# jrl-umi3218/jrl-walkgen

Measured on AMD Instinct MI355X. Metric: QP-MPC ticks/sec (batch=4096, N=16), higher is better.
Workload: dtype f64

## Files before the change

### jrl-walkgen_amd/csrc/wg_capi.hip

```cpp
#include <hip/hip_runtime.h>

#include <climits>
#include <cmath>
#include <cstdarg>
#include <cstdio>
#include <cstdlib>
#include <cstring>
#include <limits>
#include <memory>
#include <mutex>
#include <string>
#include <type_traits>
#include <vector>

#include "../../include/wg_mpc.h"
#include "wg_ql_device.hpp"
#include "wg_tick_device.hpp"
#include "wg_tick_kernels.hpp"
#include "wg_pldp_device.hpp"
#include "wg_dimitrov_device.hpp"
#include "wg_preview_device.hpp"
#include "wg_gramian_device.hpp"
#include "wg_zmpdisc_device.hpp"
#include "wg_footcons_device.hpp"
// ... 586 lines not shown
  if (!model) return fail(WG_ERR_BAD_ARG, "null model");
  if (model->N < 2 || model->N > wg::kNMaxH) return fail(WG_ERR_BAD_ARG, "N=%d outside [2,%d]", model->N, wg::kNMaxH);
  if ((int)(model->T / model->Tctrl) != WG_SAMPLES_PER_TICK)
    return fail(WG_ERR_BAD_ARG, "T/Tctrl must be %d", WG_SAMPLES_PER_TICK);
  if (tick_max_prw_steps(*model) > wg::kSMax)
    return fail(WG_ERR_BAD_ARG, "step_period=%g: a horizon of N=%d instants of T=%g previews up to %d steps, the tick holds %d",
                model->step_period, model->N, model->T, tick_max_prw_steps(*model), wg::kSMax);
  const size_t lds = TickPlan(*model).lds;
  if (lds > 160 * 1024) return fail(WG_ERR_TOO_LARGE, "tick needs %zu B of LDS > 160 KiB", lds);
  std::vector<double> qb;
  if (model->flags & (WG_FLAG_GRAMIAN_MFMA_F64 | WG_FLAG_GRAMIAN_MFMA_F32)) {
    qb.resize((size_t)model->N * model->N);
    const int prec = (model->flags & WG_FLAG_GRAMIAN_MFMA_F32) ? WG_GRAMIAN_F32 : WG_GRAMIAN_F64;
    if (int rc = wg_gramian_batch_ctx(ctx, 1, model->N, &model->T, &model->com_height_qp, model->alpha, model->beta, model->gamma,
                                  prec, qb.data()))
      return rc;
  }
  std::lock_guard<std::mutex> lk(ctx->mu);
  std::unique_ptr<wg::TickTables> host_tables_p(new wg::TickTables);
  wg::TickTables &host_tables = *host_tables_p;
  wg::build_tables(*model, host_tables, qb.empty() ? nullptr : qb.data());
  if (!host_tables.blocks_ok && !qb.empty())
    return fail(WG_ERR_BAD_ARG, "the matrix-core Gramian is not positive definite enough for ql0002's factorisation");
  if (!ctx->tables_dev) HIP_TRY(hipMalloc(reinterpret_cast<void **>(&ctx->tables_dev), sizeof(wg::TickTables)));
  if (!ctx->model_dev) HIP_TRY(hipMalloc(reinterpret_cast<void **>(&ctx->model_dev), sizeof(wg_model_t)));
  if (int rc = ctx_wait_own(ctx)) return rc;
  HostScope hs(ctx);
  WG_H2D(ctx->tables_dev, &host_tables, sizeof host_tables);
  WG_H2D(ctx->model_dev, model, sizeof(wg_model_t));
  WG_HOST_WAIT();
  ctx->model = *model;
  ctx->model_set = true;
  return WG_OK;
}

size_t wg_mpc_tick_lds_bytes_for(const wg_model_t *model) {
  if (!model || model->N < 2 || model->N > wg::kNMaxH || tick_max_prw_steps(*model) > wg::kSMax) return 0;
  return TickPlan(*model).lds;
}

size_t wg_mpc_tick_lds_bytes_ctx(wg_ctx_t *ctx) {
  if (!ctx || !ctx->model_set) return 0;
  return TickPlan(ctx->model).lds;
}

int wg_mpc_reserve_ctx(wg_ctx_t *ctx, int max_gaits) {
// ... 1380 lines not shown
```

### jrl-walkgen_amd/csrc/wg_prof.hpp

```cpp
#pragma once
#include <hip/hip_runtime.h>

namespace wg {

enum ProfSlot : int {
  PS_NORMS = 0, PS_DIAGCHK = 1, PS_CHOL = 2 , PS_INVERSE = 3,
  PS_RESID = 4, PS_ZTWW_RESID = 5, PS_XSHIFT = 6, PS_BACKSUB_RESID = 7, PS_XMAG_RESID = 8,
  PS_SCAN = 9, PS_FDIFF = 10, PS_NEWNORMAL = 11, PS_SWEEP = 12, PS_ROUTE = 13, PS_STEP_PRE = 14, PS_BACKSUB_STEP = 15,
  PS_PICKDROP = 16, PS_STEP = 17, PS_ADD = 18, PS_XMAG_ADD = 19, PS_TAIL = 20,
  PS_RESET_BODY = 24, PS_RESID_GRAD = 25, PS_RESID_FWD = 26, PS_RESID_GX = 27,
  PS_N_ROUTE = 28, PS_N_COORD = 29, PS_N_DEPENDENT = 30, PS_BORDER_ROWS = 31,
  PS_SW_NORMS = 32, PS_SW_COEFF = 33, PS_SW_ROWS = 34,
  PS_TICK_PRE = 21, PS_TICK_ASSEMBLY = 22, PS_TICK_POST = 23,
  PS_TICK_LOAD = 35, PS_TICK_FSM = 36, PS_TICK_ORIENT = 37, PS_TICK_INSTANTS = 38,
  PS_TICK_COM = 39, PS_TICK_TRUNK = 40, PS_TICK_FEET = 41, PS_TICK_QUEUE = 42,
  PS_COUNT = 48
};

#ifdef WG_PROFILE
__device__ unsigned long long g_prof[PS_COUNT];

struct PtState {
  unsigned long long acc[28] = {0}, cnt[4] = {0}, sw[3] = {0};
  unsigned long long last = clock64();
};
#define PT_DECL PtState pt;
#define PT_PARAM , PtState &pt
#define PT_ARG , pt
#define PT(k) do { unsigned long long t_ = clock64(); pt.acc[k] += t_ - pt.last; pt.last = t_; } while (0)
#define PT_VIA(k, mem, reg) do { mem = reg; PT(k); reg = mem; } while (0)
#define PT_FLUSH do { if ((threadIdx.x & 63) == 0) { for (int k_ = 0; k_ < 28; ++k_) if (k_ < PS_TICK_PRE || k_ > PS_TICK_POST) atomicAdd(&g_prof[k_], pt.acc[k_]); \
                                                      for (int k_ = 0; k_ < 4; ++k_) atomicAdd(&g_prof[PS_N_ROUTE + k_], pt.cnt[k_]); \
                                                      for (int k_ = 0; k_ < 3; ++k_) atomicAdd(&g_prof[PS_SW_NORMS + k_], pt.sw[k_]); } } while (0)
#define PT_SW_PARAM , unsigned long long *ptsw = nullptr
#define PT_SW_ARG , pt.sw
#define PT_SW(k) do { if (ptsw) { unsigned long long t_ = clock64(); ptsw[(k) - PS_SW_NORMS] += t_ - ptsw_last; ptsw_last = t_; } } while (0)
#define PT_SW_BEGIN unsigned long long ptsw_last = clock64();
#define PT_COUNT(k) do { pt.cnt[(k) - PS_N_ROUTE]++; } while (0)
#define PT_LOCAL_BEGIN unsigned long long ptl_last = clock64();
#define PT_LOCAL(k) do { unsigned long long t_ = clock64(); if ((threadIdx.x & 63) == 0) atomicAdd(&g_prof[k], t_ - ptl_last); ptl_last = t_; } while (0)

struct TkState {
  unsigned long long acc[PS_COUNT] = {0};
  unsigned long long last = clock64();
};
#define TK_DECL TkState tk;
#define TK(k) do { unsigned long long t_ = clock64(); tk.acc[k] += t_ - tk.last; tk.last = t_; } while (0)
#define TK_RESTART do { tk.last = clock64(); } while (0)
#define TK_ADD_(k) atomicAdd(&g_prof[k], tk.acc[k])
#define TK_FLUSH do { if ((threadIdx.x & 63) == 0) { const unsigned long long store_ = clock64() - tk.last; \
    TK_ADD_(PS_TICK_LOAD); TK_ADD_(PS_TICK_FSM); TK_ADD_(PS_TICK_ORIENT); TK_ADD_(PS_TICK_INSTANTS); TK_ADD_(PS_TICK_ASSEMBLY); \
    TK_ADD_(PS_TICK_COM); TK_ADD_(PS_TICK_TRUNK); TK_ADD_(PS_TICK_FEET); TK_ADD_(PS_TICK_QUEUE); \
    atomicAdd(&g_prof[PS_TICK_PRE], tk.acc[PS_TICK_LOAD] + tk.acc[PS_TICK_FSM] + tk.acc[PS_TICK_ORIENT] + tk.acc[PS_TICK_INSTANTS]); \
    atomicAdd(&g_prof[PS_TICK_POST], tk.acc[PS_TICK_COM] + tk.acc[PS_TICK_TRUNK] + tk.acc[PS_TICK_FEET] + tk.acc[PS_TICK_QUEUE] + store_); } } while (0)
#else
#define PT_DECL
#define PT_PARAM
#define PT_ARG
#define PT(k) do {} while (0)
#define PT_VIA(k, mem, reg) ((void)0)
#define PT_FLUSH do {} while (0)
#define PT_SW_PARAM
#define PT_SW_ARG
#define PT_SW(k) do {} while (0)
#define PT_SW_BEGIN
#define PT_COUNT(k) do {} while (0)
#define PT_LOCAL_BEGIN
#define PT_LOCAL(k) ((void)0)
#define TK_DECL
#define TK(k) ((void)0)
#define TK_RESTART ((void)0)
#define TK_FLUSH ((void)0)
#endif

}
```

### jrl-walkgen_amd/csrc/wg_ql_device.hpp

```cpp
#pragma once
#include <hip/hip_runtime.h>

#include <type_traits>

#include "wg_wave.hpp"
#include "wg_ql_view.hpp"
#include "wg_ql_phases.hpp"

namespace wg {

#define WG_BACKSUB(q, s, nact, lane)                                                                   \
  do {                                                                                                 \
    if constexpr (P::kNM > 0 && P::kNM + 12 <= 48) backsub_lds<48>(q, s, nact, lane, q.sc0);          \
    else if (P::kNM == 0 && (P::kWideN || q.n >= 48) && (nact) <= 60) backsub_lds<96>(q, s, nact, lane, q.sc0);     \
    else if (P::kNM == 0 && !P::kRowOps && q.n >= 24 && (nact) <= 36) backsub_lds<48>(q, s, nact, lane, q.sc0); \
    else backsub(q, s, nact, lane);                                                                    \
  } while (0)
#define WG_SWEEP(q, s, nu, nact, lane) \
  do { if (P::kNM > 0 || (!P::kRowOps && q.n <= 64)) sweep_flat<P::kFixedLdz>(q, s, nu, nact, lane PT_SW_ARG); else sweep<(P::kRowOps ? WG_ELEM_GRP : 8), P::kWideN>(q, s, nu, nact, lane); } while (0)

#define QL_SCAN_ACCEPT                                                                        \
  if (wak <= 0.0) continue;                                                                   \
  double sumx = -sum * wak;                                                                   \
  if (k + 1 <= me) sumx = fabs(sumx);                                                         \
  if (sumx <= 0.0) continue;                                                                  \
  if (bidx >= 0 && sumx <= bestv) continue;                                                   \
  double tempa = temp + fabs(sum);                                                            \
  if (tempa <= temp) continue;                                                                \
  temp += onha * fabs(sum);                                                                   \
  if (temp <= tempa) continue;                                                                \
  bestv = sumx; bestres = sum; bestw = wak; bidx = k + 1
template <class P>
__device__ __forceinline__ QlResult ql_solve(const QlView &q, P &prob, double vsmall, int *hist, int hist_cap, QlResume *rs = nullptr) {
  constexpr bool kNan = P::kNanExact && (WG_NAN_REGIME != 0);
  int lane = wg_lane();
  const int n = q.n, m = q.m, me = q.me, mn = q.mn;
  QlResult out;
  out.hist_len = 0;
  const bool resuming = rs != nullptr && rs->valid != 0;
  int nact = 0, info = 0, iterc = 1, itref = 0, iflag = 0;
  const int maxit = (m + n) * 40;
  const double onha = 1.5, xmagr = .01, diagr = 2.0;
  const int ifinc = 3, kfinc = n > 10 ? n : 10;
  int jfinc = -kfinc;
  double xmag = 0.0, vfact = 1.0, res = 0.0, ratio = 0.0, diag = 0.0;
  double wsel = 1.0;
  int knext = 0;
  const int s_tail = q.r_tail;
  double *s = q.R + s_tail;
  bool early_exit = false;
  bool cap_hit = false;
  bool x_suspect = false;
  auto x_has_non_numbers = [&]() {
    bool b = false;
    for (int i = lane; i < n; i += 64) { const bool bi = !wg_sane(q.x[i]); b = b || bi; }
    return __ballot(b) != 0ull;
  };
  PT_DECL
  if (resuming) {
    nact = rs->nact; info = rs->info; iterc = rs->iterc; itref = rs->itref; iflag = rs->iflag; jfinc = rs->jfinc; knext = rs->knext;
    out.hist_len = rs->hist_len;
    xmag = rs->xmag; vfact = rs->vfact; res = rs->res; ratio = rs->ratio; diag = rs->diag;
    if constexpr (kNan) x_suspect = x_has_non_numbers();
  }

#define LOG_EVENT(code)                                                   \
  do {                                                                    \
    if (lane == 0 && hist && out.hist_len < hist_cap) hist[out.hist_len] = (code); \
    out.hist_len++;                                                       \
  } while (0)

  if (!resuming) {
    int fatal = 0x7fffffff;
    if constexpr (P::kCompact) {
      fatal = prob.norms(q, lane);
    } else {
      for (int k = lane; k < m; k += 64) {
        double sum = 0.0;
        if constexpr (P::kRowOps) sum = prob.row_sqnorm(q, k);
        else {
          WG_UNROLL
          for (int i = 0; i < n; ++i) { double a = Am(k, i); sum += a * a; }
        }
        if (sum > 0.0) sum = 1.0 / sqrt(sum);
        else if (q.b[k] == 0.0) {}
        else if (k + 1 <= me || !(q.b[k] <= 0.0)) fatal = k + 1 < fatal ? k + 1 : fatal;
        q.wa[k] = sum;
      }
    }
    for (int k = lane; k < n; k += 64) q.wa[m + k] = 1.0;
    fatal = uni(wave_min_int(fatal));
    if (fatal != 0x7fffffff) { info = -fatal; early_exit = true; }
  }
// ... 221 lines not shown
      if (nact != n) {
        if (P::kWideN || (P::kNM == 0 && n > 64 && n <= 128)) {
          double r0, r1;
          z_rows_times<(P::kRowOps ? WG_ELEM_GRP : 8)>(q, s, nact, n, lane, r0, r1);
          q.x[lane] -= r0;
          if (lane + 64 < n) q.x[lane + 64] -= r1;
        } else
        for (int i = lane; i < n; i += 64) {
          double sum = 0.0;
          WG_UNROLL
          for (int j = nact; j < n; ++j) sum += Zm(i, j) * s[j];
          q.x[i] -= sum;
        }
        info = 0;
        WG_WSYNC();
      }
      PT(PS_XSHIFT);
      if (nact != 0) {
        WG_BACKSUB(q, s, nact, lane);
        for (int k = lane; k < nact; k += 64) q.lam[k] += q.ww[k];
        WG_WSYNC();
      }
      PT(PS_BACKSUB_RESID);
      { double sm = 0.0; WG_REP(6) { sm = uni(xmag_sum(q, prob, vfact, lane)); WG_SINK(sm); } xmag = maxd(xmag, sm); }
      PT(PS_XMAG_RESID);
      if (iflag == itref) { st = ST_RESID; continue; }
      int kd = 0x7fffffff;
      for (int k = lane; k < nact; k += 64)
        if (!(q.lam[k] >= 0.0) && q.iact[k] > me) { kd = k < kd ? k : kd; }
      kd = uni(wave_min_int(kd));
      if (kd != 0x7fffffff) {
        LOG_EVENT(-q.iact[kd]);
        nact = drop_constraint(q, kd, nact, nact, lane);
        st = ST_RESID;
        continue;
      }
      if constexpr (kNan) x_suspect = x_suspect || x_has_non_numbers();
      st = ST_SCAN;
    }

    if (st == ST_SCAN) {
      next_scan: asm volatile("" : "+v"(lane));
      double bestv = 0.0, bestres = 0.0, bestw = 0.0;
      int bidx = -1;
      if (kNan && x_suspect) {
        if constexpr (kNan) {
// ... 271 lines not shown
        else zt_times_ww<P::kNM, (P::kRowOps ? WG_ELEM_GRP : 8), P::kWideN>(q, s, lane);
      } else {
        int k1 = knext - m;
        double sg = 1.0;
        if (k1 > n) { k1 = knext - mn; sg = -1.0; }
        for (int i = lane; i < n; i += 64) {
          q.ww[i] = (i == k1 - 1) ? sg : 0.0;
          double z = Zm(k1 - 1, i);
          s[i] = (sg > 0.0) ? z : -z;
        }
        WG_WSYNC();
      }
      PT(PS_NEWNORMAL);
      double parnew = 0.0, parinc = 0.0, step = 0.0, sumy;
      int kdrop = -1;
      int route;
      if (nact == n) route = 1;
      else {
        WG_SWEEP(q, s, n, nact, lane);
        PT(PS_SWEEP);
        if (nact == 0) route = 0;
        else {
          double suma = 0.0, sumb = 0.0, sumc = 0.0;
          WG_REP(5) {
          if constexpr (P::kNM > 0) {
            constexpr int NM = P::kNM;
            {
              const int il = lane < NM ? lane : NM - 1;
              const bool in = il < n;
              const int ic = in ? il : n - 1;
              const double zv = Zm(ic, nact), wv = q.ww[ic];
              const double zi = in ? zv : 0.0, wi = in ? wv : 0.0;
              q.sc0[il] = wi * zi; q.sc1[il] = fabs(wi * zi); q.sc2[il] = zi * zi;
            }
            WG_WSYNC();
            typedef __attribute__((address_space(3))) double lds_f64;
            const lds_f64 *src = (const lds_f64 *)(q.sc0 + (lane < 3 ? lane : 0) * (int)(q.sc1 - q.sc0));
            asm volatile("" : "+v"(src));
            double acc = 0.0;
#pragma unroll
            for (int i0 = 0; i0 < NM; i0 += kOsChunk) {
              double t[kOsChunk];
#pragma unroll
              for (int i = 0; i < kOsChunk; ++i) if (i0 + i < NM) t[i] = src[i0 + i];
#pragma unroll
              for (int i = 0; i < kOsChunk; ++i) if (i0 + i < NM) acc += t[i];
            }
            suma = rl(acc, 0); sumb = rl(acc, 1); sumc = rl(acc, 2);
            WG_WSYNC();
          } else {
            for (int i = lane; i < n; i += 64) {
              const double zi = Zm(i, nact), wi = q.ww[i];
              q.sc0[i] = wi * zi; q.sc1[i] = fabs(wi * zi); q.sc2[i] = zi * zi;
            }
            WG_WSYNC();
            const double *src = q.sc0 + (lane < 3 ? lane : 0) * (int)(q.sc1 - q.sc0);
            double acc = 0.0;
            int i = 0;
            for (; i + 8 <= n; i += 8) {
              double t[8];
#pragma unroll
              for (int e = 0; e < 8; ++e) t[e] = src[i + e];
#pragma unroll
              for (int e = 0; e < 8; ++e) acc += t[e];
            }
            for (; i < n; ++i) acc += src[i];
            suma = rl(acc, 0); sumb = rl(acc, 1); sumc = rl(acc, 2);
            WG_WSYNC();
          }
          WG_SINK(suma); WG_SINK(sumb); WG_SINK(sumc);
          }
          if (WG_UBOOL(!significant(sumb, fabs(suma)) || !(sumb > wg_kconst(vsmall)))) route = 1;
          else {
            sumc = sqrt(sumc);
            if (knext <= m) sumc /= wsel;
            if (WG_UBOOL(significant(sumc, fabs(suma)))) route = 0;
            else {
              PT_COUNT(PS_N_COORD);
              WG_BACKSUB(q, s, nact, lane);
              route = independent_coordinate(q, prob, knext, nact, vsmall, lane) ? 0 : 2;
            }
          }
        }
      }
      route = uni(route);
      PT(PS_ROUTE);
      PT_COUNT(PS_N_ROUTE);
      if (route != 0) PT_COUNT(PS_N_DEPENDENT);
      if (route != 0) {
        if (route == 1) WG_BACKSUB(q, s, nact, lane);
        kdrop = pick_drop<(P::kNM > 0), kNan>(q, nact, res, ratio, lane);
        info = -knext;
        if (kdrop < 0) { st = ST_CONVERGED; continue; }
        parinc = ratio;
        parnew = parinc;
// ... 49 lines not shown
          LOG_EVENT(-q.iact[kdrop]);
          nact = drop_constraint(q, kdrop, nu, nact, lane);
          double *snew = s - (nact + 1);
          if (nu > n) nu = n;
          for (int i0 = 0; i0 < nu; i0 += 64) {
            int i = i0 + lane;
            double v = (i < nu) ? s[i] : 0.0;
            WG_WSYNC();
            if (i < nu) snew[i] = v;
            WG_WSYNC();
          }
          s = snew;
          WG_SWEEP(q, s, nu, nact, lane);
        }
      }

      PT(PS_STEP);
      ql_activate(q, nact, knext, parnew, wsel, lane, n, mn);
      nact++;
      LOG_EVENT(knext);
      WG_WSYNC();
      PT(PS_ADD);
      double sm = 0.0;
      WG_REP(6) { sm = uni(xmag_sum(q, prob, vfact, lane)); WG_SINK(sm); }
      xmag = maxd(xmag, sm);
      PT(PS_XMAG_ADD);
      if (WG_UBOOL(sm < wg_kconst(xmagr) * xmag)) st = ST_RESET;
      else if (itref <= 0) st = ST_SCAN;
      else st = ST_RESID;
      if (q.nact_cap > 0 && nact > q.nact_cap) { cap_hit = true; break; }
      if (st == ST_SCAN) goto next_scan;
      continue;
    }

    if (st == ST_CONVERGED) {
      ++itref;
      jfinc = -1;
      if (itref == 1) { st = ST_RESID; continue; }
      st = ST_FINISH;
    }
  }
#undef LOG_EVENT

  PT(PS_TAIL);
  PT_FLUSH;
  if (cap_hit) {
    if (rs) {
      rs->nact = nact; rs->info = info; rs->iterc = iterc; rs->itref = itref; rs->iflag = iflag; rs->jfinc = jfinc; rs->knext = knext;
      rs->st = st; rs->hist_len = out.hist_len;
      rs->xmag = xmag; rs->vfact = vfact; rs->res = res; rs->ratio = ratio; rs->diag = diag;
    }
    out.ifail = kQlCapHit; out.n_iter = iterc; out.nact = nact;
    return out;
  }
  out.ifail = ql_ifail_of(info);
  out.n_iter = iterc;
  out.nact = nact;
  return out;
}

}
```

### jrl-walkgen_amd/csrc/wg_ql_herdt.hpp

```cpp
#pragma once
#include "wg_ql_device.hpp"

namespace wg {

constexpr int kSMaxQ = 4;
constexpr int kGvLd = 4;
constexpr int kQbLd = 32;

template <int NH, int NS>
__device__ __forceinline__ bool herdt_border_rows(const QlView &q, const double *gd, const double *Gv, double vsmall, int lane) {
  constexpr int M2 = 2 * NH;
  const int i = lane;
  const bool jerk = i < NH, foot = i >= NH && i < NH + NS, row = jerk || foot;
  const int fi = i - NH;
  const int gi = jerk ? i : M2 + (foot ? fi : 0);
  double acc[NS];
#pragma unroll
  for (int f = 0; f < NS; ++f)
    acc[f] = (jerk || (foot && f >= fi)) ? ((foot && f == fi) ? gd[gi] : Gv[gi * kGvLd + f]) : 0.0;
  const double dreg = jerk ? Rf(i, i) : 1.0;
  const int colbase = jerk ? i * (i + 1) / 2 : 0;
  const int khi = jerk ? i : 0;
  double rnext = (0 < khi) ? q.Rf[colbase] : 0.0;
  for (int k = 0; k < NH; ++k) {
// ... 152 lines not shown
#pragma unroll
  for (int t = 0; t < TZ; ++t) {
    const int e = lane + 64 * t;
    if (e < NH * NH) {
      const int i = e % NH, j = e / NH;
      Zm(i, j) = zv[t]; Zm(NH + i, NH + j) = zv[t];
      Zm(NH + i, j) = 0.0;
      Zm(i, NH + j) = ((z2sign[e >> 6] >> (e & 63)) & 1ull) ? wg_kconst(-0.0) : 0.0;
    }
  }
  for (int e = lane; e < (n - M2) * M2; e += 64) { const int i = M2 + e % (n - M2), j = e / (n - M2); Zm(i, j) = 0.0; }
}

template <int NH>
struct HerdtProb {
  static constexpr bool kCompact = true;
  static constexpr bool kNanExact = WG_TICK_NAN_EXACT != 0;
  static constexpr bool kHasFactor = true;
  static constexpr bool kRowOps = false;
  static constexpr int kNM = 2 * NH + 2 * 2;
  static constexpr int kCopRows = 4 * NH;
  static constexpr bool kWideN = false;
  static constexpr int kFixedLdz = kNM | 1;
  static_assert(4 * NH == 64, "one CoP row per lane needs 4N == 64");
  const double *Qb;
  const double *u;
  double *Gv;
  double *gd;
  const double *rowA, *rowB;
  const int *rowK, *stepidx;
  const double *V_f;
  const double *R2, *Z2;
  const unsigned long long *z2sign;
  double diag_b;
  int blocks_ok;
  int ns;
  double ax[NH], ay[NH];
  int fj;
  double ra, rb;
  double bcop;
  double ga, gb; int gk;
  __device__ __forceinline__ double fa() const { return ra + 0.0; }
  __device__ __forceinline__ double fb() const { return rb + 0.0; }
  struct FootRow { double v[4]; int c[4]; };
  __device__ __forceinline__ FootRow foot_row() const {
    const bool used = gk >= 0, pred = gk > 0;
    const int kk = used ? gk : 0;
    FootRow r;
    const int c1 = 2 * NH + kk, c3 = 2 * NH + ns + kk;
    r.c[0] = used ? (pred ? c1 - 1 : c1) : 2 * NH; r.c[1] = used ? c1 : 2 * NH;
    r.c[2] = used ? (pred ? c3 - 1 : c3) : 2 * NH; r.c[3] = used ? c3 : 2 * NH;
    r.v[0] = pred ? ga + 0.0 : 0.0; r.v[1] = used ? 0.0 - ga : 0.0;
    r.v[2] = pred ? gb + 0.0 : 0.0; r.v[3] = used ? 0.0 - gb : 0.0;
    return r;
  }

  __device__ __forceinline__ double G(const QlView &q, int i, int j) const {
    if (i == j) return gd[i];
    if (j < i) { const int t = i; i = j; j = t; }
// ... 511 lines not shown
```

### jrl-walkgen_amd/csrc/wg_ql_phases.hpp

```cpp
#pragma once
#include <hip/hip_runtime.h>

#include <type_traits>

#include "wg_wave.hpp"
#include "wg_ql_view.hpp"

namespace wg {

#ifndef WG_ELEM_GRP
#define WG_ELEM_GRP 4
#endif

__device__ __forceinline__ double sqrt_1to2(double x) {
  const double y = __builtin_amdgcn_rsq(x);
  double g = x * y;
  double h = y * 0.5;
  const double r = __builtin_fma(-h, g, 0.5);
  g = __builtin_fma(g, r, g);
  h = __builtin_fma(h, r, h);
  double d = __builtin_fma(-g, g, x);
  g = __builtin_fma(d, h, g);
  d = __builtin_fma(-g, g, x);
  g = __builtin_fma(d, h, g);
// ... 322 lines not shown


#ifndef WG_OS_CHUNK
#define WG_OS_CHUNK 12
#endif
constexpr int kOsChunk = WG_OS_CHUNK;
template <int NM>
__device__ __forceinline__ double ordered_sum_lds(double term, double *scratch, int cnt, int lane) {
  {
    const double v = (lane < cnt) ? term : 0.0;
    const double vl = rl(v, NM - 1);
    scratch[lane < NM ? lane : NM - 1] = lane < NM ? v : vl;
  }
  WG_WSYNC();
  double sum = 0.0;
#pragma unroll
  for (int i0 = 0; i0 < NM; i0 += kOsChunk) {
    double t[kOsChunk];
#pragma unroll
    for (int i = 0; i < kOsChunk; ++i) t[i] = (i0 + i < NM) ? scratch[i0 + i] : 0.0;
#pragma unroll
    for (int i = 0; i < kOsChunk; ++i) if (i0 + i < NM) sum += t[i];
  }
  WG_WSYNC();
  return sum;
}

template <int kLdzC = 0>
__device__ __forceinline__ void sweep_flat(const QlView &q, double *s, int nu, int nact, int lane PT_SW_PARAM) {
  const int n = q.n;
  if (nu - 1 <= nact) return;
  PT_SW_BEGIN
  double *chain = q.sc2;
  WG_REP(3)
  if (sweep_range_ok<true>(s, nact, nu, lane)) {
    double cur = s[nu - 1];
    double pa = s[nu - 2], pb;
    int c = nu - 1;
    typedef __attribute__((address_space(3))) double lds_f64;
    const lds_f64 *sp = (const lds_f64 *)(s + (nu - 4));
    lds_f64 *cp = (lds_f64 *)(chain + (nu - 3));
    asm volatile("" : "+v"(sp), "+v"(cp));
    const int rots = c - nact;
    if (WG_UBOOL(cur != 0.0)) {
      for (int k = rots >> 1; k > 0; --k) {
        pb = sp[1];
// ... 398 lines not shown
    const int il = lane < n ? lane : n - 1;
    const double xi = q.x[il];
    const double term = fabs(xi) * vfact * (fabs(q.d[il]) + fabs(prob.Gd(q, il) * xi));
    return ordered_sum_lds<P::kNM>(term, q.sc3, n, lane);
  }
  for (int i = lane; i < n; i += 64) {
    double xi = q.x[i];
    q.sc3[i] = fabs(xi) * vfact * (fabs(q.d[i]) + fabs(prob.Gd(q, i) * xi));
  }
  WG_WSYNC();
  double sum = 0.0;
  int i = 0;
  for (; i + 8 <= n; i += 8) {
    double t[8];
#pragma unroll
    for (int e = 0; e < 8; ++e) t[e] = q.sc3[i + e];
#pragma unroll
    for (int e = 0; e < 8; ++e) sum += t[e];
  }
  for (; i < n; ++i) sum += q.sc3[i];
  return sum;
}

template <int GRP = 8, bool kWide = false>
__device__ __forceinline__ void sweep(const QlView &q, double *s, int nu, int nact, int lane) {
  const int n = q.n;
  if (nu - 1 <= nact) return;
  if (!kWide && n <= 64) {
    const double sreg = (lane < nu) ? s[lane] : 0.0;
    double myP = 0.0, myQ = 0.0, myN = 0.0;
    {
      double cur = rl(sreg, nu - 1);
      for (int c = nu - 1; c > nact; --c) {
        const double p = rl(sreg, c - 1);
        double nrm;
        if (cur == 0.0) { nrm = 0.0; cur = p; }
        else { nrm = givens_norm(p, cur); if (lane == c) { myP = p; myQ = cur; } cur = nrm; }
        if (lane == c) myN = nrm;
      }
    }
    double ga = 1.0, gb = 0.0;
    if (lane > nact && lane < nu && myN != 0.0) {
      ga = myP / myN;
      gb = myQ / myN;
      s[lane - 1] = myN;
    }
// ... 321 lines not shown
```

### jrl-walkgen_amd/csrc/wg_ql_view.hpp

```cpp
#pragma once
#include <hip/hip_runtime.h>

#include <type_traits>

#include "wg_wave.hpp"
#include "wg_prof.hpp"

namespace wg {

struct QlDims {
  int n, m, mmax;
  int ldg, ldz, lda;
  bool dense;
  bool a_lds;
  int nsc;
  bool bounds;
  bool z_lds;
  bool wab_lds;
  bool cold_lds;
  int r_cols;
  bool g_lds;
  __host__ __device__ QlDims(int n_, int m_, int mmax_, bool dense_ = true, bool a_lds_ = true, int nsc_ = 0,
                             bool bounds_ = true, bool z_lds_ = true, bool wab_lds_ = true, bool cold_lds_ = true, int r_cols_ = 0,
                             bool g_lds_ = true)
// ... 143 lines not shown
#pragma unroll
      for (int i = 0; i < NM; ++i)
        if (i < n) dst[i] = k < 64 ? ar0[i] : ar1[i];
    }
  }
};
template <class P, class = void> struct HasRegRows { static constexpr bool value = false; };
template <class P> struct HasRegRows<P, typename std::enable_if<P::kRegRows>::type> { static constexpr bool value = true; };
#define Rp(i, j) q.R[(j) * ((j) + 1) / 2 + (i)]
#define Rf(i, j) q.Rf[(j) * ((j) + 1) / 2 + (i)]

#ifdef WG_REPEAT_PHASE
#define WG_REP(id) for (int wg_rep_ = 0; wg_rep_ < (((WG_REPEAT_PHASE) == (id)) ? 2 : 1); ++wg_rep_, ({ asm volatile("" ::: "memory"); }))
#define WG_SINK(x) asm volatile("" ::"v"(x))
#else
#define WG_REP(id)
#define WG_SINK(x) do {} while (0)
#endif

struct NoActiveParams {};
template <class P, class = void> struct ActiveParamsOf { typedef NoActiveParams type; };
template <class P> struct ActiveParamsOf<P, typename std::enable_if<P::kCompact>::type> { typedef typename P::ActiveParams type; };

struct QlResult {
  int ifail, n_iter, nact, hist_len;
};
struct QlResume {
  int valid = 0;
  int nact, info, iterc, itref, iflag, jfinc, knext, st, hist_len;
  double xmag, vfact, res, ratio, diag;
};

template <bool kGLds, int kNMc> __device__ __forceinline__ double DenseProbT<kGLds, kNMc>::G(const QlView &q, int i, int j) const {
  if constexpr (kGLds) return q.G[i + j * q.ldg];
  else {
    const double g = q.G[i + j * q.ldg], dg = q.Gdiag[i];
    return i == j ? dg : g;
  }
}
template <bool kGLds, int kNMc> __device__ __forceinline__ double DenseProbT<kGLds, kNMc>::A(const QlView &q, int k, int i) const { return q.A[k + i * q.lda]; }
template <bool kGLds, int kNMc> __device__ __forceinline__ double DenseProbT<kGLds, kNMc>::Gd(const QlView &q, int i) const {
  if constexpr (kGLds) return q.G[i + i * q.ldg]; else return q.Gdiag[i];
}
template <bool kGLds, int kNMc> __device__ __forceinline__ void DenseProbT<kGLds, kNMc>::setGd(const QlView &q, int i, double v) const {
  if constexpr (kGLds) q.G[i + i * q.ldg] = v; else q.Gdiag[i] = v;
}
// ... 5 lines not shown
```

### jrl-walkgen_amd/csrc/wg_tick_device.hpp

```cpp
#pragma once
#include <hip/hip_runtime.h>

#include <cmath>

#include "../../include/wg_mpc.h"
#define WG_TRIG_FN __host__ __device__ static inline
#include "../../include/wg_trig.h"
#include "wg_ql_device.hpp"
#include "wg_ql_herdt.hpp"

namespace wg {

#define GmL(i, j) q.G[(i) + (j) * q.ldg]
#define AmL(k, i) q.A[(k) + (i) * q.lda]
#define WG_STATE_COPY(to, from)                                                                                       \
  { double *dst = reinterpret_cast<double *>(to); const double *src = reinterpret_cast<const double *>(from);          \
    for (int i = lane; i < (int)(sizeof(wg_gait_state_t) / 8); i += 64) dst[i] = src[i]; }
#define WG_STATE_COPY_LD(to, from, scope)                                                                              \
  { const double *src = reinterpret_cast<const double *>(from); double *dst = reinterpret_cast<double *>(to);           \
    for (int i = lane; i < (int)(sizeof(wg_gait_state_t) / 8); i += 64) dst[i] = __hip_atomic_load(src + i, __ATOMIC_RELAXED, scope); }

constexpr int kNMaxH = 32;
constexpr int kSMax = 4;
constexpr double kPi = 3.14159265358979323846;

struct TickTables {
  double Sv[kNMaxH][3], Sz[kNMaxH][3];
  double Uv[kNMaxH][kNMaxH], Uz[kNMaxH][kNMaxH];
  double Qb[kNMaxH][kNMaxH];
  double R2[2 * kNMaxH * (2 * kNMaxH + 1) / 2];
  double Z2[4 * kNMaxH * kNMaxH];
  double diag_b;
  int blocks_ok, pad_;
  unsigned long long z2_cross_sign[(kNMaxH * kNMaxH + 63) / 64];
};

inline void build_tables(const wg_model_t &m, TickTables &t, const double *qb_override = nullptr) {
  const int N = m.N;
  const double T = m.T, h = m.com_height_qp;
  for (unsigned i = 0; i < (unsigned)kNMaxH; i++)
    for (unsigned j = 0; j < (unsigned)kNMaxH; j++) { t.Uv[i][j] = 0.0; t.Uz[i][j] = 0.0; t.Qb[i][j] = 0.0; }
  for (unsigned i = 0; i < (unsigned)N; i++) {
    t.Sv[i][0] = 0.0; t.Sv[i][1] = 1.0; t.Sv[i][2] = (i + 1) * T;
    t.Sz[i][0] = 1.0; t.Sz[i][1] = (i + 1) * T;
    t.Sz[i][2] = (i + 1) * (i + 1) * T * T * 0.5 - h / 9.81;
    for (unsigned j = 0; j <= i; j++) {
      t.Uv[i][j] = (2 * (i - j) + 1) * T * T * 0.5;
      t.Uz[i][j] = (1 + 3 * (i - j) + 3 * (i - j) * (i - j)) * T * T * T / 6.0 - T * h / 9.81;
    }
  }
  for (int i = 0; i < N; i++)
    for (int j = 0; j < N; j++) {
      double pj = 0.0, pv = 0.0, pz = 0.0;
      for (int k = 0; k < N; k++) {
        pj += ((k == i) ? 1.0 : 0.0) * ((k == j) ? 1.0 : 0.0);
        pv += t.Uv[k][i] * t.Uv[k][j];
// ... 7 lines not shown
    }
  {
    const int M = 2 * N;
    const double vsmall = 1e-8;
    auto g2 = [&](int i, int j) -> double {
      if (i < N && j < N) return t.Qb[i][j];
      if (i >= N && j >= N) return t.Qb[i - N][j - N];
      return 0.0;
    };
    double diag = 0.0;
    for (int i = 0; i < M; ++i) {
      const double wdi = g2(i, i);
      diag = (diag >= vsmall - wdi) ? diag : vsmall - wdi;
      for (int j = i + 1; j < M; ++j) {
        const double gjj = g2(j, j), gij = g2(i, j);
        double ga = -((wdi <= gjj) ? wdi : gjj);
        const double gb = fabs(wdi - gjj) + fabs(gij);
        if (gb > 0.0) ga += gij * gij / gb;
        diag = (diag >= ga) ? diag : ga;
      }
    }
    t.diag_b = diag;
    t.blocks_ok = (diag <= 0.0) ? 1 : 0;
    t.pad_ = 0;
    auto R = [&](int i, int j) -> double & { return t.R2[(size_t)j * (j + 1) / 2 + i]; };
    for (int j = 0; j < M && t.blocks_ok; ++j) {
      double temp = 0.0;
      for (int i = 0; i <= j; ++i) {
        temp = g2(i, j);
        for (int k = 0; k < i; ++k) temp -= R(k, j) * R(k, i);
        if (i < j) R(i, j) = temp / R(i, i);
      }
      if (temp < vsmall) { t.blocks_ok = 0; break; }
      R(j, j) = sqrt(temp);
    }
    auto Z = [&](int i, int j) -> double & { return t.Z2[(size_t)i + (size_t)j * M]; };
    if (t.blocks_ok)
      for (int i = 0; i < M; ++i) {
        for (int j = 0; j < i; ++j) Z(i, j) = 0.0;
        Z(i, i) = 1.0 / R(i, i);
        for (int j = i; j < M - 1; ++j) {
          double sum = 0.0;
          for (int k = i; k <= j; ++k) sum += Z(i, k) * R(k, j + 1);
          Z(i, j + 1) = -sum / R(j + 1, j + 1);
        }
      }
    for (auto &w : t.z2_cross_sign) w = 0ull;
// ... 655 lines not shown
            AmL(r, 2 * N + j) = 0.0 + px * -1.0; AmL(r, 2 * N + ns + j) = 0.0 + py * -1.0;
          }
        }
        bacc += L.rowD[r];
        bacc += (0.0 + a * L.Vc_fX[k]) * 1.0;
        bacc += (0.0 + bb * L.Vc_fY[k]) * 1.0;
      }
    }
    q.b[r] = -bacc;
  }
  WG_WSYNC();
  }

  TK(PS_TICK_ASSEMBLY);
  QlResult qr;
  if constexpr (kCompactView) {
    if (lane == 0 && fabs(L.gd[n - 1]) == 0.0) L.gd[n - 1] = wg_kconst(1e-8);
    WG_WSYNC();
    WG_STATE_COPY(gstate, s);
    HerdtProb<16> prob;
    prob.Qb = &tb->Qb[0][0]; prob.u = L.uvec; prob.Gv = L.Gv; prob.gd = L.gd;
    prob.rowA = L.rowA; prob.rowB = L.rowB; prob.rowK = L.rowK; prob.stepidx = L.stepidx; prob.V_f = L.V_f;
    prob.R2 = tb->R2; prob.Z2 = tb->Z2; prob.z2sign = tb->z2_cross_sign; prob.diag_b = tb->diag_b; prob.blocks_ok = tb->blocks_ok; prob.ns = ns;
    prob.load_rows(lane, q.b);
    qr = ql_solve(q, prob, 1e-8, hist, hist_cap);
    {
      WG_WSYNC();
      __builtin_amdgcn_fence(__ATOMIC_RELEASE, "workgroup");
      WG_STATE_COPY_LD(s, gstate, __HIP_MEMORY_SCOPE_AGENT);
      WG_WSYNC();
    }
  } else if constexpr (kElem) {
    if (lane == 0 && fabs(L.gd[n - 1]) == 0.0) L.gd[n - 1] = 1e-8;
    WG_WSYNC();
    {
      WG_STATE_COPY(gstate, s);
      __builtin_amdgcn_fence(__ATOMIC_RELEASE, "workgroup");
    }
    HerdtElemProbT<(NH == 32) ? 32 : -1> prob;
    prob.N = N; prob.ns = ns; prob.Qb = &tb->Qb[0][0]; prob.u = L.uvec; prob.Gv = L.Gv; prob.gd = L.gd;
    prob.rowA = L.rowA; prob.rowB = L.rowB; prob.rowK = L.rowK; prob.stepidx = L.stepidx; prob.V_f = L.V_f;
    prob.R2 = tb->R2; prob.Z2 = tb->Z2; prob.z2sign = tb->z2_cross_sign; prob.blocks_ok = tb->blocks_ok;
    QlResume rs;
    qr = ql_solve(q, prob, 1e-8, hist, hist_cap, &rs);
    if (WG_UBOOL(qr.ifail == kQlCapHit)) {
      WG_WSYNC();
      double *Rg = extE + eRfull;
      const int cnt = qr.nact * (qr.nact + 1) / 2;
// ... 248 lines not shown
```

### jrl-walkgen_amd/csrc/wg_wave.hpp

```cpp
#pragma once
#include <hip/hip_runtime.h>

namespace wg {

#ifndef WG_UNROLL_N
#define WG_UNROLL_N 4
#endif
#define WG_PRAGMA(x) _Pragma(#x)
#define WG_UNROLL_(n) WG_PRAGMA(unroll n)
#define WG_UNROLL WG_UNROLL_(WG_UNROLL_N)

#define WG_WSYNC()                                          \
  do {                                                      \
    __builtin_amdgcn_fence(__ATOMIC_RELEASE, "wavefront");  \
    __builtin_amdgcn_wave_barrier();                        \
    __builtin_amdgcn_fence(__ATOMIC_ACQUIRE, "wavefront");  \
  } while (0)

__device__ __forceinline__ int wg_lane() { int l = threadIdx.x & 63; asm volatile("" : "+v"(l)); return l; }
__device__ __forceinline__ int uni(int v) { return __builtin_amdgcn_readfirstlane(v); }
__device__ __forceinline__ double uni(double v) {
  int lo = __double2loint(v), hi = __double2hiint(v);
  lo = __builtin_amdgcn_readfirstlane(lo);
  hi = __builtin_amdgcn_readfirstlane(hi);
// ... 37 lines not shown
  v = __builtin_fmax(v, dpp_keep<0x118>(v));
  v = __builtin_fmax(v, dpp_keep<0x142>(v));
  v = __builtin_fmax(v, dpp_keep<0x143>(v));
  return rl(v, 63);
}
__device__ __forceinline__ int wave_min_int(int v) {
  { const int o = dpp_keep<0x111>(v); v = o < v ? o : v; }
  { const int o = dpp_keep<0x112>(v); v = o < v ? o : v; }
  { const int o = dpp_keep<0x114>(v); v = o < v ? o : v; }
  { const int o = dpp_keep<0x118>(v); v = o < v ? o : v; }
  { const int o = dpp_keep<0x142>(v); v = o < v ? o : v; }
  { const int o = dpp_keep<0x143>(v); v = o < v ? o : v; }
  return __builtin_amdgcn_readlane(v, 63);
}
__device__ __forceinline__ int wave_max_int(int v) {
  { const int o = dpp_keep<0x111>(v); v = o > v ? o : v; }
  { const int o = dpp_keep<0x112>(v); v = o > v ? o : v; }
  { const int o = dpp_keep<0x114>(v); v = o > v ? o : v; }
  { const int o = dpp_keep<0x118>(v); v = o > v ? o : v; }
  { const int o = dpp_keep<0x142>(v); v = o > v ? o : v; }
  { const int o = dpp_keep<0x143>(v); v = o > v ? o : v; }
  return __builtin_amdgcn_readlane(v, 63);
}
__device__ __forceinline__ void wave_argmax_first(double &v, int &idx) {
  const double vv = idx >= 0 ? v : -__builtin_huge_val();
  const double vmax = wave_max(vv);
  const int key = (idx >= 0 && v == vmax) ? idx : 0x7fffffff;
  const int kmin = wave_min_int(key);
  v = vmax;
  idx = kmin == 0x7fffffff ? -1 : kmin;
}

}
```

Before: 6.817 million.

## Use guarded tree reductions in QL step and xmag sums with ordered-sum rerun fallback

In the Herdt QL solver, the step-length sums and the xmag sums now use fast DPP tree reductions instead of serial ordered sums. Certified error bounds check whether the decision taken from the tree result would match the one from the sequential-order sum. When a decision cannot be certified, the solve restarts in ordered mode, so results stay bit-compatible with the reference at the cost of occasional full reruns. An environment variable can force ordered or doubt mode, and profiling counters for fallbacks and reruns are added.

```diff
diff --git a/jrl-walkgen_amd/csrc/wg_capi.hip b/jrl-walkgen_amd/csrc/wg_capi.hip
--- a/jrl-walkgen_amd/csrc/wg_capi.hip
+++ b/jrl-walkgen_amd/csrc/wg_capi.hip
@@ -632,6 +632,12 @@
   wg::build_tables(*model, host_tables, qb.empty() ? nullptr : qb.data());
   if (!host_tables.blocks_ok && !qb.empty())
     return fail(WG_ERR_BAD_ARG, "the matrix-core Gramian is not positive definite enough for ql0002's factorisation");
+  if (const char *e = getenv("WG_QL_SUMS")) {
+    const std::string v(e);
+    if (v == "ordered") host_tables.ql_sums = wg::kSumsOrdered;
+    else if (v == "doubt") host_tables.ql_sums = wg::kSumsDoubt;
+    else if (!v.empty() && v != "guarded") return fail(WG_ERR_BAD_ARG, "WG_QL_SUMS=%s: ordered, doubt or unset", e);
+  }
   if (!ctx->tables_dev) HIP_TRY(hipMalloc(reinterpret_cast<void **>(&ctx->tables_dev), sizeof(wg::TickTables)));
   if (!ctx->model_dev) HIP_TRY(hipMalloc(reinterpret_cast<void **>(&ctx->model_dev), sizeof(wg_model_t)));
   if (int rc = ctx_wait_own(ctx)) return rc;
diff --git a/jrl-walkgen_amd/csrc/wg_prof.hpp b/jrl-walkgen_amd/csrc/wg_prof.hpp
--- a/jrl-walkgen_amd/csrc/wg_prof.hpp
+++ b/jrl-walkgen_amd/csrc/wg_prof.hpp
@@ -14,6 +14,7 @@
   PS_TICK_PRE = 21, PS_TICK_ASSEMBLY = 22, PS_TICK_POST = 23,
   PS_TICK_LOAD = 35, PS_TICK_FSM = 36, PS_TICK_ORIENT = 37, PS_TICK_INSTANTS = 38,
   PS_TICK_COM = 39, PS_TICK_TRUNK = 40, PS_TICK_FEET = 41, PS_TICK_QUEUE = 42,
+  PS_N_FALLBACK = 43, PS_N_RERUN = 44,
   PS_COUNT = 48
 };
 
@@ -21,7 +22,7 @@
 __device__ unsigned long long g_prof[PS_COUNT];
 
 struct PtState {
-  unsigned long long acc[28] = {0}, cnt[4] = {0}, sw[3] = {0};
+  unsigned long long acc[28] = {0}, cnt[4] = {0}, sw[3] = {0}, cnt2[2] = {0};
   unsigned long long last = clock64();
 };
 #define PT_DECL PtState pt;
@@ -31,12 +32,14 @@
 #define PT_VIA(k, mem, reg) do { mem = reg; PT(k); reg = mem; } while (0)
 #define PT_FLUSH do { if ((threadIdx.x & 63) == 0) { for (int k_ = 0; k_ < 28; ++k_) if (k_ < PS_TICK_PRE || k_ > PS_TICK_POST) atomicAdd(&g_prof[k_], pt.acc[k_]); \
                                                       for (int k_ = 0; k_ < 4; ++k_) atomicAdd(&g_prof[PS_N_ROUTE + k_], pt.cnt[k_]); \
-                                                      for (int k_ = 0; k_ < 3; ++k_) atomicAdd(&g_prof[PS_SW_NORMS + k_], pt.sw[k_]); } } while (0)
+                                                      for (int k_ = 0; k_ < 3; ++k_) atomicAdd(&g_prof[PS_SW_NORMS + k_], pt.sw[k_]); \
+                                                      for (int k_ = 0; k_ < 2; ++k_) atomicAdd(&g_prof[PS_N_FALLBACK + k_], pt.cnt2[k_]); } } while (0)
 #define PT_SW_PARAM , unsigned long long *ptsw = nullptr
 #define PT_SW_ARG , pt.sw
 #define PT_SW(k) do { if (ptsw) { unsigned long long t_ = clock64(); ptsw[(k) - PS_SW_NORMS] += t_ - ptsw_last; ptsw_last = t_; } } while (0)
 #define PT_SW_BEGIN unsigned long long ptsw_last = clock64();
 #define PT_COUNT(k) do { pt.cnt[(k) - PS_N_ROUTE]++; } while (0)
+#define PT_COUNT2(k) do { pt.cnt2[(k) - PS_N_FALLBACK]++; } while (0)
 #define PT_LOCAL_BEGIN unsigned long long ptl_last = clock64();
 #define PT_LOCAL(k) do { unsigned long long t_ = clock64(); if ((threadIdx.x & 63) == 0) atomicAdd(&g_prof[k], t_ - ptl_last); ptl_last = t_; } while (0)
 
@@ -65,6 +68,7 @@
 #define PT_SW(k) do {} while (0)
 #define PT_SW_BEGIN
 #define PT_COUNT(k) do {} while (0)
+#define PT_COUNT2(k) do {} while (0)
 #define PT_LOCAL_BEGIN
 #define PT_LOCAL(k) ((void)0)
 #define TK_DECL
diff --git a/jrl-walkgen_amd/csrc/wg_ql_device.hpp b/jrl-walkgen_amd/csrc/wg_ql_device.hpp
--- a/jrl-walkgen_amd/csrc/wg_ql_device.hpp
+++ b/jrl-walkgen_amd/csrc/wg_ql_device.hpp
@@ -6,6 +6,9 @@
 #include "wg_wave.hpp"
 #include "wg_ql_view.hpp"
 #include "wg_ql_phases.hpp"
+#define WG_GUARD_FN __device__ __forceinline__
+#define WG_GUARD_K(c) ::wg::wg_kconst(c)
+#include "wg_ql_guard.hpp"
 
 namespace wg {
 
@@ -33,6 +36,9 @@
 template <class P>
 __device__ __forceinline__ QlResult ql_solve(const QlView &q, P &prob, double vsmall, int *hist, int hist_cap, QlResume *rs = nullptr) {
   constexpr bool kNan = P::kNanExact && (WG_NAN_REGIME != 0);
+  constexpr bool kGuard = GuardedSumsOf<P>::value;
+  [[maybe_unused]] int gmode = kSumsOrdered;
+  if constexpr (kGuard) gmode = uni(prob.sums_mode);
   int lane = wg_lane();
   const int n = q.n, m = q.m, me = q.me, mn = q.mn;
   QlResult out;
@@ -69,6 +75,15 @@
     if (lane == 0 && hist && out.hist_len < hist_cap) hist[out.hist_len] = (code); \
     out.hist_len++;                                                       \
   } while (0)
+#define QL_RERUN_ORDERED                                                              \
+  do {                                                                                \
+    PT_COUNT2(PS_N_RERUN);                                                            \
+    for (int i = lane; i < n; i += 64) prob.setGd(q, i, q.wd[i]);                     \
+    WG_WSYNC();                                                                       \
+    PT_FLUSH;                                                                         \
+    out.ifail = kQlDoubt; out.n_iter = iterc; out.nact = nact;                        \
+    return out;                                                                       \
+  } while (0)
 
   if (!resuming) {
     int fatal = 0x7fffffff;
@@ -336,6 +351,12 @@
         WG_WSYNC();
       }
       PT(PS_BACKSUB_RESID);
+      if constexpr (kGuard) {
+        double sm = 0.0;
+        WG_REP(6) { sm = uni(xmag_sum_guarded(q, prob, vfact, lane, gmode == kSumsOrdered)); WG_SINK(sm); }
+        if (gmode != kSumsOrdered && WG_UBOOL(x_suspect || !guard_xmag_update(sm))) QL_RERUN_ORDERED;
+        xmag = maxd(xmag, sm);
+      } else
       { double sm = 0.0; WG_REP(6) { sm = uni(xmag_sum(q, prob, vfact, lane)); WG_SINK(sm); } xmag = maxd(xmag, sm); }
       PT(PS_XMAG_RESID);
       if (iflag == itref) { st = ST_RESID; continue; }
@@ -653,8 +674,43 @@
         if (nact == 0) route = 0;
         else {
           double suma = 0.0, sumb = 0.0, sumc = 0.0;
+          bool step_certain = false;
           WG_REP(5) {
-          if constexpr (P::kNM > 0) {
+          if constexpr (kGuard) {
+            constexpr int NM = P::kNM;
+            static_assert(NM > 32 && NM <= 48, "three entries per lane of a 16-lane row");
+            {
+              const int il = lane < NM ? lane : NM - 1;
+              const bool in = il < n;
+              const int ic = in ? il : n - 1;
+              const double zv = Zm(ic, nact), wv = q.ww[ic];
+              const double zi = in ? zv : 0.0, wi = in ? wv : 0.0;
+              q.sc0[il] = wi * zi; q.sc1[il] = fabs(wi * zi); q.sc2[il] = zi * zi;
+            }
+            WG_WSYNC();
+            if (gmode == kSumsGuarded && !x_suspect) {
+              const int row = (lane >> 4) < 3 ? (lane >> 4) : 2, j = lane & 15;
+              const int j2 = j + 32 < NM ? j + 32 : NM - 1;
+              const double *vec = q.sc0 + row * (int)(q.sc1 - q.sc0);
+              const double t0 = vec[j], t1 = vec[j + 16], t2 = vec[j2];
+              double v = (t0 + t1) + (j + 32 < NM ? t2 : 0.0);
+              v += dpp_zero<0x111, 0xf>(v);
+              v += dpp_zero<0x112, 0xf>(v);
+              v += dpp_zero<0x114, 0xf>(v);
+              v += dpp_zero<0x118, 0xf>(v);
+              suma = rl(v, 15); sumb = rl(v, 31); sumc = rl(v, 47);
+              step_certain = WG_UBOOL(guard_route0(suma, sumb, sumc, knext <= m, wsel, wg_kconst(vsmall)));
+            }
+            if (!step_certain) {
+              if (gmode != kSumsOrdered) PT_COUNT2(PS_N_FALLBACK);
+              const double *src = q.sc0 + (lane < 3 ? lane : 0) * (int)(q.sc1 - q.sc0);
+              double acc = 0.0;
+#pragma nounroll
+              for (int i = 0; i < NM; ++i) acc += src[i];
+              suma = rl(acc, 0); sumb = rl(acc, 1); sumc = rl(acc, 2);
+            }
+            WG_WSYNC();
+          } else if constexpr (P::kNM > 0) {
             constexpr int NM = P::kNM;
             {
               const int il = lane < NM ? lane : NM - 1;
@@ -701,7 +757,8 @@
           }
           WG_SINK(suma); WG_SINK(sumb); WG_SINK(sumc);
           }
-          if (WG_UBOOL(!significant(sumb, fabs(suma)) || !(sumb > wg_kconst(vsmall)))) route = 1;
+          if (kGuard && step_certain) route = 0;
+          else if (WG_UBOOL(!significant(sumb, fabs(suma)) || !(sumb > wg_kconst(vsmall)))) route = 1;
           else {
             sumc = sqrt(sumc);
             if (knext <= m) sumc /= wsel;
@@ -797,12 +854,28 @@
       WG_WSYNC();
       PT(PS_ADD);
       double sm = 0.0;
+      if constexpr (kGuard) {
+        WG_REP(6) { sm = uni(xmag_sum_guarded(q, prob, vfact, lane, gmode == kSumsOrdered)); WG_SINK(sm); }
+        xmag = maxd(xmag, sm);
+        PT(PS_XMAG_ADD);
+        bool reset;
+        if (gmode == kSumsOrdered) reset = WG_UBOOL(sm < wg_kconst(xmagr) * xmag);
+        else {
+          const int verdict = x_suspect ? (int)kGuardDoubt : uni(guard_xmag(sm, xmag));
+          if (verdict == kGuardDoubt) QL_RERUN_ORDERED;
+          reset = verdict == kGuardReset;
+        }
+        if (reset) st = ST_RESET;
+        else if (itref <= 0) st = ST_SCAN;
+        else st = ST_RESID;
+      } else {
       WG_REP(6) { sm = uni(xmag_sum(q, prob, vfact, lane)); WG_SINK(sm); }
       xmag = maxd(xmag, sm);
       PT(PS_XMAG_ADD);
       if (WG_UBOOL(sm < wg_kconst(xmagr) * xmag)) st = ST_RESET;
       else if (itref <= 0) st = ST_SCAN;
       else st = ST_RESID;
+      }
       if (q.nact_cap > 0 && nact > q.nact_cap) { cap_hit = true; break; }
       if (st == ST_SCAN) goto next_scan;
       continue;
@@ -815,6 +888,8 @@
       st = ST_FINISH;
     }
   }
+  if constexpr (kGuard) { if (gmode == kSumsDoubt && !early_exit && !cap_hit) QL_RERUN_ORDERED; }
+#undef QL_RERUN_ORDERED
 #undef LOG_EVENT
 
   PT(PS_TAIL);
@@ -834,4 +909,16 @@
   return out;
 }
 
+template <class P>
+__device__ __forceinline__ QlResult ql_solve_guarded(const QlView &q, P &prob, double vsmall, int *hist, int hist_cap) {
+  static_assert(GuardedSumsOf<P>::value, "for policies with kGuardedSums");
+  QlResult r;
+  for (;;) {
+    r = ql_solve(q, prob, vsmall, hist, hist_cap);
+    if (!WG_UBOOL(r.ifail == kQlDoubt)) break;
+    prob.sums_mode = kSumsOrdered;
+  }
+  return r;
 }
+
+}
diff --git a/jrl-walkgen_amd/csrc/wg_ql_guard.hpp b/jrl-walkgen_amd/csrc/wg_ql_guard.hpp
--- /dev/null
+++ b/jrl-walkgen_amd/csrc/wg_ql_guard.hpp
@@ -0,0 +1,57 @@
+#pragma once
+#include <cmath>
+
+#ifndef WG_GUARD_FN
+#define WG_GUARD_FN inline
+#endif
+#ifndef WG_GUARD_K
+#define WG_GUARD_K(c) (c)
+#endif
+
+namespace wg {
+
+enum GuardVerdict : int { kGuardDoubt = -1, kGuardNoReset = 0, kGuardReset = 1 };
+
+WG_GUARD_FN bool guard_route0(double suma, double sumb, double sumc, bool by_wa, double wa, double vsmall) {
+  const double big = WG_GUARD_K(0x1p500);
+  const double as = std::fabs(suma);
+  if (!(as < big) || !(sumb < big) || !(sumc < big)) return false;
+  if (!(sumb * WG_GUARD_K(1.0 - 0x1p-46) > vsmall)) return false;
+  const double d = as - WG_GUARD_K(0x1p-46) * sumb;
+  if (!(d >= WG_GUARD_K(0x1p-40 * (1.0 + 0x1p-40)) * sumb)) return false;
+  double p = d;
+  if (by_wa) {
+    if (!(wa > 0.0)) return false;
+    p = d * wa;
+  }
+  if (!(p >= WG_GUARD_K(0x1p-400))) return false;
+  return p * p >= WG_GUARD_K(0x1p-80 * (1.0 + 0x1p-39 + 0x1p-52)) * sumc;
+}
+
+WG_GUARD_FN int guard_xmag(double s, double xmag) {
+  const double big = WG_GUARD_K(0x1p500);
+  if (!(s > 0.0) || !(s < big) || !(xmag < big)) return kGuardDoubt;
+  const double t = WG_GUARD_K(.01) * xmag;
+  if (s >= t * WG_GUARD_K(1.0 + 0x1p-40)) return kGuardNoReset;
+  if (s <= t * WG_GUARD_K(1.0 - 0x1p-40)) return kGuardReset;
+  return kGuardDoubt;
+}
+
+WG_GUARD_FN bool guard_xmag_update(double s) { return s < WG_GUARD_K(0x1p500); }
+
+inline double guard_tree_sum(const double *t, int n) {
+  double v[64];
+  for (int i = 0; i < 64; ++i) v[i] = i < n ? t[i] : 0.0;
+  for (int w = 1; w < 64; w *= 2)
+    for (int i = 0; i < 64; i += 2 * w) v[i] = v[i + w] + v[i];
+  return v[0];
+}
+inline double guard_rows_sum(const double *t, int n) {
+  double v[16];
+  for (int j = 0; j < 16; ++j) v[j] = ((j < n ? t[j] : 0.0) + (j + 16 < n ? t[j + 16] : 0.0)) + (j + 32 < n ? t[j + 32] : 0.0);
+  for (int w = 1; w < 16; w *= 2)
+    for (int i = 0; i < 16; i += 2 * w) v[i] = v[i + w] + v[i];
+  return v[0];
+}
+
+}
diff --git a/jrl-walkgen_amd/csrc/wg_ql_herdt.hpp b/jrl-walkgen_amd/csrc/wg_ql_herdt.hpp
--- a/jrl-walkgen_amd/csrc/wg_ql_herdt.hpp
+++ b/jrl-walkgen_amd/csrc/wg_ql_herdt.hpp
@@ -198,6 +198,7 @@
   static constexpr int kCopRows = 4 * NH;
   static constexpr bool kWideN = false;
   static constexpr int kFixedLdz = kNM | 1;
+  static constexpr bool kGuardedSums = true;
   static_assert(4 * NH == 64, "one CoP row per lane needs 4N == 64");
   const double *Qb;
   const double *u;
@@ -211,6 +212,7 @@
   double diag_b;
   int blocks_ok;
   int ns;
+  int sums_mode;
   double ax[NH], ay[NH];
   int fj;
   double ra, rb;
diff --git a/jrl-walkgen_amd/csrc/wg_ql_phases.hpp b/jrl-walkgen_amd/csrc/wg_ql_phases.hpp
--- a/jrl-walkgen_amd/csrc/wg_ql_phases.hpp
+++ b/jrl-walkgen_amd/csrc/wg_ql_phases.hpp
@@ -368,6 +368,21 @@
 #pragma unroll
     for (int i = 0; i < kOsChunk; ++i) if (i0 + i < NM) sum += t[i];
   }
+  WG_WSYNC();
+  return sum;
+}
+
+template <int NM>
+__device__ __forceinline__ double ordered_sum_lds_rolled(double term, double *scratch, int cnt, int lane) {
+  {
+    const double v = (lane < cnt) ? term : 0.0;
+    const double vl = rl(v, NM - 1);
+    scratch[lane < NM ? lane : NM - 1] = lane < NM ? v : vl;
+  }
+  WG_WSYNC();
+  double sum = 0.0;
+#pragma nounroll
+  for (int i = 0; i < NM; ++i) sum += scratch[i];
   WG_WSYNC();
   return sum;
 }
@@ -812,6 +827,16 @@
   return sum;
 }
 
+template <class P>
+__device__ __forceinline__ double xmag_sum_guarded(const QlView &q, const P &prob, double vfact, int lane, bool ordered) {
+  const int n = q.n;
+  const int il = lane < n ? lane : n - 1;
+  const double xi = q.x[il];
+  const double term = fabs(xi) * vfact * (fabs(q.d[il]) + fabs(prob.Gd(q, il) * xi));
+  if (ordered) return ordered_sum_lds_rolled<P::kNM>(term, q.sc3, n, lane);
+  return wave_sum_tree(lane < n ? term : 0.0);
+}
+
 template <int GRP = 8, bool kWide = false>
 __device__ __forceinline__ void sweep(const QlView &q, double *s, int nu, int nact, int lane) {
   const int n = q.n;
diff --git a/jrl-walkgen_amd/csrc/wg_ql_view.hpp b/jrl-walkgen_amd/csrc/wg_ql_view.hpp
--- a/jrl-walkgen_amd/csrc/wg_ql_view.hpp
+++ b/jrl-walkgen_amd/csrc/wg_ql_view.hpp
@@ -189,6 +189,11 @@
 template <class P, class = void> struct ActiveParamsOf { typedef NoActiveParams type; };
 template <class P> struct ActiveParamsOf<P, typename std::enable_if<P::kCompact>::type> { typedef typename P::ActiveParams type; };
 
+template <class P, class = void> struct GuardedSumsOf { static constexpr bool value = false; };
+template <class P> struct GuardedSumsOf<P, typename std::enable_if<P::kGuardedSums>::type> { static constexpr bool value = true; };
+enum : int { kSumsGuarded = 0, kSumsOrdered = 1, kSumsDoubt = 2 };
+constexpr int kQlDoubt = -7778;
+
 struct QlResult {
   int ifail, n_iter, nact, hist_len;
 };
diff --git a/jrl-walkgen_amd/csrc/wg_tick_device.hpp b/jrl-walkgen_amd/csrc/wg_tick_device.hpp
--- a/jrl-walkgen_amd/csrc/wg_tick_device.hpp
+++ b/jrl-walkgen_amd/csrc/wg_tick_device.hpp
@@ -31,7 +31,8 @@
   double R2[2 * kNMaxH * (2 * kNMaxH + 1) / 2];
   double Z2[4 * kNMaxH * kNMaxH];
   double diag_b;
-  int blocks_ok, pad_;
+  int blocks_ok;
+  int ql_sums;
   unsigned long long z2_cross_sign[(kNMaxH * kNMaxH + 63) / 64];
 };
 
@@ -85,7 +86,7 @@
     }
     t.diag_b = diag;
     t.blocks_ok = (diag <= 0.0) ? 1 : 0;
-    t.pad_ = 0;
+    t.ql_sums = 0;
     auto R = [&](int i, int j) -> double & { return t.R2[(size_t)j * (j + 1) / 2 + i]; };
     for (int j = 0; j < M && t.blocks_ok; ++j) {
       double temp = 0.0;
@@ -787,8 +788,9 @@
     prob.Qb = &tb->Qb[0][0]; prob.u = L.uvec; prob.Gv = L.Gv; prob.gd = L.gd;
     prob.rowA = L.rowA; prob.rowB = L.rowB; prob.rowK = L.rowK; prob.stepidx = L.stepidx; prob.V_f = L.V_f;
     prob.R2 = tb->R2; prob.Z2 = tb->Z2; prob.z2sign = tb->z2_cross_sign; prob.diag_b = tb->diag_b; prob.blocks_ok = tb->blocks_ok; prob.ns = ns;
+    prob.sums_mode = tb->ql_sums;
     prob.load_rows(lane, q.b);
-    qr = ql_solve(q, prob, 1e-8, hist, hist_cap);
+    qr = ql_solve_guarded(q, prob, 1e-8, hist, hist_cap);
     {
       WG_WSYNC();
       __builtin_amdgcn_fence(__ATOMIC_RELEASE, "workgroup");
diff --git a/jrl-walkgen_amd/csrc/wg_wave.hpp b/jrl-walkgen_amd/csrc/wg_wave.hpp
--- a/jrl-walkgen_amd/csrc/wg_wave.hpp
+++ b/jrl-walkgen_amd/csrc/wg_wave.hpp
@@ -83,6 +83,21 @@
   { const int o = dpp_keep<0x143>(v); v = o > v ? o : v; }
   return __builtin_amdgcn_readlane(v, 63);
 }
+template <int CTRL, int ROWS>
+__device__ __forceinline__ double dpp_zero(double v) {
+  const int lo = __builtin_amdgcn_update_dpp(0, __double2loint(v), CTRL, ROWS, 0xf, true);
+  const int hi = __builtin_amdgcn_update_dpp(0, __double2hiint(v), CTRL, ROWS, 0xf, true);
+  return __hiloint2double(hi, lo);
+}
+__device__ __forceinline__ double wave_sum_tree(double v) {
+  v += dpp_zero<0x111, 0xf>(v);
+  v += dpp_zero<0x112, 0xf>(v);
+  v += dpp_zero<0x114, 0xf>(v);
+  v += dpp_zero<0x118, 0xf>(v);
+  v += dpp_zero<0x142, 0xa>(v);
+  v += dpp_zero<0x143, 0xc>(v);
+  return rl(v, 63);
+}
 __device__ __forceinline__ void wave_argmax_first(double &v, int &idx) {
   const double vv = idx >= 0 ? v : -__builtin_huge_val();
   const double vmax = wave_max(vv);
```

Result: faster. 6.915 million, median of 6 (+1.4%).
